# classicvalues/foremast

Measured on AMD Instinct MI355X. Metric: metric windows scored/sec (node) + p50 decision latency, 10k-service canary, higher is better.
Workload: dtype fp32; 1 GPU; global_batch=80000, seq_len=10080, services=10000, metrics=8, current_points_per_window=50, parallelism=dp1, hip_graph=False, tick_mode=front, decision_stream=comm (overlaps next front kernel), front_wgs_per_cu=1:4, comm_overlap=decision + all-gather + host copy of tick k on a comm stream || tick k+1, pipeline_depth=2, publish=graph

## Files before the change

csrc/include/fm_pairwise.h:

```cpp
#pragma once
#include "fm_common.h"

using namespace fm;

namespace {

constexpr float kPad = INFINITY;

template <int K, bool SPLIT = false, bool TAGGED = true, typename T>
__device__ __forceinline__ void bitonic_sort(T (&v)[K], int (&tag)[K]) {
  static_assert(!SPLIT || (K == 2 && TAGGED), "split layout is two tagged 64-lane registers");
  const int lane = lane_id();
#pragma unroll
  for (int size = 2; size <= 64 * K; size <<= 1) {
    const bool tags = TAGGED && (!SPLIT || size > 64);
    if constexpr (SPLIT) {
      if (size == 128) {
#pragma unroll
        for (int k = 0; k < K; ++k) tag[k] = v[k] == kPad ? -1 : k;
      }
    }
#pragma unroll
    for (int stride = size >> 1; stride > 0; stride >>= 1) {
      if (stride >= 64) {
        const int ks = stride / 64;
#pragma unroll
        for (int k = 0; k < K; ++k) {
          const int p = k ^ ks;
          if (p > k) {
// ... 3 lines not shown
            const bool first = (a < b) == asc;
            v[k] = first ? a : b; v[p] = first ? b : a;
            if (tags) {
              const int ta = tag[k], tb = tag[p];
              tag[k] = first ? ta : tb; tag[p] = first ? tb : ta;
            }
          }
        }
      } else {
#pragma unroll
        for (int k = 0; k < K; ++k) {
          const int i = k * 64 + lane;
          const bool asc = (i & size) == 0;
          const bool lower = (lane & stride) == 0;
          const bool keep_min = lower == asc;
          if (tags) cmpx_lane_any(v[k], tag[k], stride, keep_min);
          else cmpx_lane_any(v[k], stride, keep_min);
        }
      }
    }
  }
}

template <int K, bool REDUCE, typename T>
__device__ __forceinline__ int avg_ranks(const T (&v)[K], int n, int (&rank2)[K], bool (&is_end)[K]) {
  const int lane = lane_id();
  bool ne_prev[K];
  unsigned long long tied = 0;
  T last_prev = 0;
#pragma unroll
  for (int k = 0; k < K; ++k) {
    const T prev = lane_prev(v[k], last_prev);
// ... 95 lines not shown
  o[5] = (n1 > 0 && n2 > 0) ? (double)dnum / ((double)n1 * n2) : 0.0;
  o[6] = 0.5 * (double)rps; o[7] = (double)tiew; o[8] = m1; o[9] = m2; o[10] = q1; o[11] = q2;
  o[12] = npos; o[13] = nzero;
}

struct PwNoHook {
  __device__ __forceinline__ void loaded() const {}
  __device__ __forceinline__ void done() const {}
  __device__ __forceinline__ void store(double* __restrict__ o, int n1, int n2, int nw, unsigned r1s, unsigned tie,
                                        int dnum, unsigned rps, unsigned tiew, float m1, float m2, float q1, float q2,
                                        int npos, int nzero) const {
    if (lane_id() == 0) pw_store_suff(o, n1, n2, nw, r1s, tie, dnum, rps, tiew, m1, m2, q1, q2, npos, nzero);
  }
};

template <int K, bool SPLIT = false, class Hook = PwNoHook>
__device__ __forceinline__ void pw_compute(PwIn<K>& in, int n_cur, int n_base, double* __restrict__ o,
                                           Hook hook = Hook()) {
  const int lane = lane_id();
  float (&v)[K] = in.v;
  int tag[K];
  float s1 = 0.f, s2 = 0.f;
  int n1 = 0, n2 = 0;
#pragma unroll
  for (int k = 0; k < K; ++k) {
    const int i = k * 64 + lane;
    int t = SPLIT ? (lane < (k == 0 ? n_cur : n_base) ? k : -1) : (i < n_cur ? 0 : (i < n_cur + n_base ? 1 : -1));
    float x = v[k];
    if (!isfinite(x)) { x = kPad; t = -1; }
    v[k] = x; tag[k] = t;
    if (t == 0) s1 += x;
    if (t == 1) s2 += x;
    n1 += __popcll(__ballot(t == 0));
    n2 += __popcll(__ballot(t == 1));
  }
  const int n = n1 + n2;
  const float m1 = wave_sum_f32_uniform(s1) / (float)(n1 > 0 ? n1 : 1);
  const float m2 = wave_sum_f32_uniform(s2) / (float)(n2 > 0 ? n2 : 1);
  float q1 = 0.f, q2 = 0.f;
#pragma unroll
  for (int k = 0; k < K; ++k) {
    if (tag[k] == 0) { const float d = v[k] - m1; q1 += d * d; }
    if (tag[k] == 1) { const float d = v[k] - m2; q2 += d * d; }
  }
  q1 = wave_sum_f32_uniform(q1); q2 = wave_sum_f32_uniform(q2);

  constexpr int KW = PwIn<K>::KW;
  constexpr unsigned kPadMag = 0x7F800000u;
  unsigned dk[KW];
  const int npair = n_cur < n_base ? n_cur : n_base;
  int nw = 0, npos = 0, nzero = 0;
#pragma unroll
  for (int k = 0; k < KW; ++k) {
    const int j = k * 64 + lane;
    const float xc = in.pc[k], xb = in.pb[k];
    const float dd = xc - xb;
    const bool ok = j < npair && isfinite(xc) && isfinite(xb);
    const bool nz = ok && dd != 0.f, pos = nz && dd > 0.f;
    dk[k] = nz ? ((__float_as_uint(fabsf(dd)) << 1) | (pos ? 1u : 0u)) : (kPadMag << 1);
    nw += __popcll(__ballot(nz));
    npos += __popcll(__ballot(pos));
    nzero += __popcll(__ballot(ok && !nz));
  }

  hook.loaded();
  constexpr long long N = 64LL * K, NW = 64LL * KW;
  constexpr int bTie = pw_bits(N * N * N - N), bR1 = pw_bits(N * (N + 1));
  constexpr int bTiew = pw_bits(NW * NW * NW - NW), bRp = pw_bits(NW * (NW + 1));
  static_assert(bTie <= 32 && bTiew <= 32 && bR1 <= 32 && bRp <= 32, "32-bit sums");
  constexpr bool packA = bTie + bR1 <= 32;
  constexpr bool packB = bTiew + bRp <= 32;
  constexpr bool packC = !packA && !packB && bR1 + bRp <= 32;
  bitonic_sort<K, SPLIT>(v, tag);
  int rk2[K];
  bool en[K];
  const int tie_l = avg_ranks<K, !packA>(v, n, rk2, en);

  unsigned r1x2 = 0;
  int dnum = 0;
  int base12 = 0;
#pragma unroll
  for (int k = 0; k < K; ++k) {
    if (tag[k] == 0) r1x2 += (unsigned)rk2[k];
    const int a12 = wave_incl_sum(tag[k] == 0 ? 1 : (tag[k] == 1 ? (1 << 16) : 0)) + base12;
    base12 = lane_bcast(a12, 63);
    if (en[k] && n1 > 0 && n2 > 0) {
      const int a1 = a12 & 0xFFFF, a2 = a12 >> 16;
      const int dd = abs(__mul24(a1, n2) - __mul24(a2, n1));
// ... 286 lines not shown
```

csrc/kernels/tick_front.hip:

```cpp
#include "fm_pairwise.h"
#include "fm_row_stats.h"

__device__ __attribute__((noinline)) void eval_test_call(int t, const double* __restrict__ o, int min_mw, int min_wil,
                                                         int min_kru, double& pv, double& sv) {
  eval_test(t, o, min_mw, min_wil, min_kru, pv, sv);
}

#ifdef FM_FRONT_TIMING
constexpr int kFtMarks = 4;
__device__ unsigned long long g_front_t[kFtMarks * 8192];
#define FM_FT_MARK(k) \
  do { if (threadIdx.x == 0 && blockIdx.x < 8192) g_front_t[kFtMarks * blockIdx.x + (k)] = __builtin_amdgcn_s_memrealtime(); } while (0)
#define FM_FT_ROWS(n) \
  do { if (threadIdx.x == 0 && blockIdx.x < 8192) g_front_t[kFtMarks * blockIdx.x + 3] = (unsigned long long)(n); } while (0)
#else
#define FM_FT_MARK(k) do {} while (0)
#define FM_FT_ROWS(n) do {} while (0)
#endif

struct FrontArgs {
  int64_t R;
  int nP, scan, T;
  const float* hist;
  int64_t ld_h;
  float* hs;
  const int* rowmap;
  float* cache;
  unsigned* valid;
  unsigned* queue;
  const float* cur;
  int64_t ld_c;
  const float* base;
  int64_t ld_b;
  double* suff;
  int n_cur, n_base;
  float *pvals, *pstats;
  int min_mw, min_wil, min_kru;
};

constexpr int kXcdCtl = 256, kCtlR = 0, kCtlDone = 1, kCtlB = 2, kCtlOn = 31, kCtlT0 = 32, kCtlT1 = 48;
constexpr int64_t kXcdMinRows = 32768;
constexpr int kFracBits = 24;
constexpr double kXcdBand = 1.015, kXcdStep = 3.0;
constexpr int kHistChunk = 1;
__device__ inline int64_t xcd_bound(int64_t R, unsigned f) { return (R * (int64_t)f) >> kFracBits; }

__device__ __attribute__((noinline)) void xcd_rebalance(unsigned* ctl, int xcd, int64_t R) {
  unsigned long long* t0 = reinterpret_cast<unsigned long long*>(ctl + kCtlT0);
  unsigned long long* t1 = reinterpret_cast<unsigned long long*>(ctl + kCtlT1);
  __hip_atomic_store(t1 + xcd, __builtin_amdgcn_s_memrealtime(), __ATOMIC_RELAXED, __HIP_MEMORY_SCOPE_AGENT);
  const unsigned g = __hip_atomic_fetch_add(ctl + kCtlDone, 1u, __ATOMIC_ACQ_REL, __HIP_MEMORY_SCOPE_AGENT);
  if (g != 7u) return;
// ... 70 lines not shown
      uint4* s = reinterpret_cast<uint4*>(raw);
      s[0] = make_uint4((unsigned)n1, (unsigned)n2, (unsigned)nw, r1s);
      s[1] = make_uint4(tie, (unsigned)dnum, rps, tiew);
      s[2] = make_uint4(__float_as_uint(m1), __float_as_uint(m2), __float_as_uint(q1), __float_as_uint(q2));
      *reinterpret_cast<uint2*>(raw + 12) = make_uint2((unsigned)npos, (unsigned)nzero);
    }
  }
};

__device__ __forceinline__ void front_raw_to_suff(const unsigned* __restrict__ raw, double* __restrict__ o) {
  const uint4 a = reinterpret_cast<const uint4*>(raw)[0], b = reinterpret_cast<const uint4*>(raw)[1];
  const uint4 c = reinterpret_cast<const uint4*>(raw)[2];
  const uint2 d = *reinterpret_cast<const uint2*>(raw + 12);
  pw_store_suff(o, (int)a.x, (int)a.y, (int)a.z, a.w, b.x, (int)b.y, b.z, b.w, __uint_as_float(c.x),
                __uint_as_float(c.y), __uint_as_float(c.z), __uint_as_float(c.w), (int)d.x, (int)d.y);
}

template <int K>
__device__ __forceinline__ void pw_row_grab(const float* __restrict__ c, const float* __restrict__ b, int n_cur,
                                            int n_base, unsigned* raw, bool want, unsigned* ctr, unsigned& next) {
  PwIn<K> in;
  if constexpr (K == 2) {
    if (n_cur <= 64 && n_base <= 64) {
      pw_load<K, true>(c, b, n_cur, n_base, in);
      pw_compute<K, true>(in, n_cur, n_base, nullptr, PwGrab{ctr, want, next, raw});
      return;
    }
  }
  pw_load<K>(c, b, n_cur, n_base, in);
  pw_compute<K, false>(in, n_cur, n_base, nullptr, PwGrab{ctr, want, next, raw});
// ... 8 lines not shown
    const int ci = (u >> 1) * 8 + ((u & 1) ? 7 - slot : slot);
    if (ci >= N_TESTS * cpt) break;
    const int tp = ci / cpt;
    const int t = __builtin_amdgcn_readfirstlane((int)((kByCost >> (4 * tp)) & 7u));
    const int j = (ci - tp * cpt) * 64 + lane_id();
    const int64_t row = j < nr ? rowOf(j) : -1;
    if (row >= 0) {
      double pv, sv;
      eval_test_call(t, a.suff + row * kSuff, a.min_mw, a.min_wil, a.min_kru, pv, sv);
      a.pvals[row * N_TESTS + t] = (float)pv;
      a.pstats[row * N_TESTS + t] = (float)sv;
    }
  }
}

template <int K>
__device__ __forceinline__ void front_pairwise_static(const FrontArgs& a, const int pb) {
  const int64_t R = a.R, first = (int64_t)pb * 4, stride = (int64_t)a.nP * 4;
  for (int64_t row = first + wave_id(); row < R; row += stride) {
    pw_row<K>(a.cur + row * a.ld_c, a.base + row * a.ld_b, a.n_cur, a.n_base, a.suff + row * kSuff);
  }
  __syncthreads();
  FM_FT_MARK(2);
  const int64_t span = R > first ? R - first : 0;
  const int nr = (int)(((span + stride - 1) / stride) * 4);
#ifdef FM_FRONT_TIMING
  {
    int64_t took = 0;
    for (int w = 0; w < 4; ++w) took += span > w ? (span - w + stride - 1) / stride : 0;
    FM_FT_ROWS(took);
  }
#endif
  front_pvalues(a, nr, (wave_id() + pb) & 3, [&](int j) {
    const int64_t row = first + (j & 3) + (int64_t)(j >> 2) * stride;
    return row < R ? row : (int64_t)-1;
  });
}

template <int K>
__device__ __forceinline__ void front_pairwise_dyn(const FrontArgs& a, const FrontDyn& dq, const int pb) {
  __shared__ int s_rows[4][kRowCap];
  __shared__ int s_cnt[4];
  __shared__ __attribute__((aligned(16))) unsigned s_raw[4][kRowCap][kRawWords];
  const int w = wave_id(), lane = lane_id();
  const int nP = a.nP, W = nP * 4, Q = dq.q;
  const int x = (pb + pb / Q) % Q;
  const int64_t pool = a.R - dq.pool0;
  const int lo = dq.pool0 + (int)(pool * x / Q), hi = dq.pool0 + (int)(pool * (x + 1) / Q);
  const unsigned nx = (unsigned)(hi - lo);
  unsigned* ctr = dq.pq + x * 32;
  unsigned next = 0;
  bool pending = false;
  if (dq.s == 0 && nx != 0u) {
    unsigned idx = 0;
// ... 7 lines not shown
    int row;
    if (i < dq.s) {
      row = pb * 4 + w + i * W;
    } else {
      if (!pending) break;
      if (next >= nx) break;
      row = lo + (int)next;
    }
    switch ((cls + i) & 3) {
      case 0: __builtin_amdgcn_s_setprio(0); break;
      case 1: __builtin_amdgcn_s_setprio(1); break;
      case 2: __builtin_amdgcn_s_setprio(2); break;
      default: __builtin_amdgcn_s_setprio(3); break;
    }
    const bool want = nx != 0u && i + 1 >= dq.s && i + 1 < kRowCap;
    pw_row_grab<K>(a.cur + (int64_t)row * a.ld_c, a.base + (int64_t)row * a.ld_b, a.n_cur, a.n_base, s_raw[w][i],
                   want, ctr, next);
    pending = want;
    if (lane == 0) s_rows[w][i] = row;
    ++i;
  }
  __builtin_amdgcn_s_setprio(0);
  if (lane == 0) s_cnt[w] = i;
  __syncthreads();
  FM_FT_MARK(2);
  const int c0 = s_cnt[0], c1 = c0 + s_cnt[1], c2 = c1 + s_cnt[2], nr = c2 + s_cnt[3];
  FM_FT_ROWS(nr);
  auto listed = [&](int j, int& ww, int& k) {
    ww = (j >= c0 ? 1 : 0) + (j >= c1 ? 1 : 0) + (j >= c2 ? 1 : 0);
    k = j - (ww == 0 ? 0 : (ww == 1 ? c0 : (ww == 2 ? c1 : c2)));
  };
  if ((int)threadIdx.x < nr) {
// ... 70 lines not shown
    __syncthreads();
    if (threadIdx.x == 0) s_next = nxt;
    __syncthreads();
    r0 = lo + (int64_t)s_next;
  }
  if (threadIdx.x == 0) {
    const unsigned d = atomicAdd(ctr + 1, 1u);
    if (d == (unsigned)nwg - 1) {
      __hip_atomic_store(ctr, 0u, __ATOMIC_RELAXED, __HIP_MEMORY_SCOPE_AGENT);
      __hip_atomic_store(ctr + 1, 0u, __ATOMIC_RELAXED, __HIP_MEMORY_SCOPE_AGENT);
      if (bal) xcd_rebalance(ctl, xcd, R);
    }
  }
}

template <int NV, int K, bool DYN>
__device__ __forceinline__ void tick_front_body(const FrontArgs& a, const FrontDyn& dq) {
  __shared__ double red[4];
  __shared__ int redi[4];
  FM_FT_MARK(0);
  const int nH = (int)gridDim.x - a.nP;
  const int pb = DYN ? (int)blockIdx.x - nH : (int)blockIdx.x;
  const int64_t hb = DYN ? (int64_t)blockIdx.x : (int64_t)blockIdx.x - a.nP;
  if (pb >= 0 && pb < a.nP) {
    if constexpr (DYN) front_pairwise_dyn<K>(a, dq, pb);
    else front_pairwise_static<K>(a, pb);
  } else if (DYN || a.scan) {
    front_hist_scan<NV>(a, hb, nH, red, redi);
  } else if (a.queue == nullptr) {
    front_hist_stride<NV>(a.hist, a.ld_h, a.T, a.R, a.hs, a.rowmap, a.cache, a.valid, hb, nH, red, redi);
  } else {
    front_hist_queue<NV>(a.hist, a.ld_h, a.T, a.R, a.hs, a.rowmap, a.cache, a.valid, a.queue, hb, nH, red, redi);
  }
  FM_FT_MARK(1);
}

template <int NV, int K>
__global__ __launch_bounds__(256) void tick_front_kernel(const FrontArgs a) {
  tick_front_body<NV, K, false>(a, FrontDyn{});
}

template <int NV, int K>
__global__ __launch_bounds__(256) void tick_front_dyn_kernel(const FrontArgs a, const FrontDyn dq) {
  tick_front_body<NV, K, true>(a, dq);
}

struct FrontPlan {
  int nP, s, q;
  int64_t pool0;
};
static FrontPlan front_plan(int64_t R, int nP, int q_ranges, bool scan) {
  static const int share = [] {
    const char* e = getenv("FM_FRONT_DYN_SHARE");
    const int v = e != nullptr ? atoi(e) : -1;
    return v < 0 || v > 100 ? -1 : v;
  }();
  const int64_t pmax = (R + 3) / 4;
  if (nP <= 0 || nP > pmax) nP = (int)pmax;
  const int64_t per0 = R > 0 ? (R + 4 * (int64_t)nP - 1) / (4 * (int64_t)nP) : 0;
// ... 15 lines not shown
FM_API int fm_front_plan(int64_t R, int nP, int q_ranges, int scan, int64_t* out) {
  if (out == nullptr) return (int)hipErrorInvalidValue;
  const FrontPlan p = front_plan(R, nP, q_ranges, scan != 0);
  out[0] = p.s, out[1] = p.pool0, out[2] = p.q, out[3] = p.nP;
  return 0;
}

static unsigned front_lds() {
  static const unsigned b = [] {
    const char* e = getenv("FM_FRONT_LDS");
    return e != nullptr ? (unsigned)atoi(e) : 33u * 1024u;
  }();
  return b;
}

FM_API int fm_tick_front(const float* hist, int64_t ld_h, int T, int64_t R, float* hs, const float* cur, int64_t ld_c,
                         int n_cur, const float* base, int64_t ld_b, int n_base, double* suff, int nP, int nH,
                         int min_mw, int min_wil, int min_kru, float* pvals, float* pstats, unsigned* queue,
                         const int* rowmap, float* cache, unsigned* valid, int expect_miss, unsigned* pqueue,
                         int q_ranges, hipStream_t stream) {
  if (R <= 0) return 0;
  if ((ld_h & 3) != 0 || (((uintptr_t)hist) & 15) != 0) return (int)hipErrorInvalidValue;
  const int n = n_cur + n_base;
  if (base == nullptr || n_base <= 0 || n > 256) return (int)hipErrorInvalidValue;
  if (cache == nullptr || valid == nullptr || T <= 0) cache = nullptr, valid = nullptr;
  const int scan = cache != nullptr && expect_miss == 0 ? 1 : 0;
  const FrontPlan plan = front_plan(R, nP, pqueue != nullptr ? q_ranges : 0, scan != 0);
  if (scan && nH <= 0) nH = (int)((R + 255) / 256);
  if (nH <= 0 || nH > R) nH = (int)R;
  if (!scan && queue != nullptr && nH < 8) nH = 8;
  const int nq = (T + 3) / 4;
  const dim3 grid((unsigned)(plan.nP + nH)), block(256);
  const unsigned lds = scan ? 0u : front_lds();
  const FrontArgs a{R, plan.nP, scan, T, hist, ld_h, hs, rowmap, cache, valid, queue, cur, ld_c, base, ld_b, suff,
                    n_cur, n_base, pvals, pstats, min_mw, min_wil, min_kru};
  const FrontDyn dq{pqueue, plan.q, plan.s, (int)plan.pool0};
  const int rc = row_stats_dispatch_nv(nq, [&](auto nv) {
    auto launch = [&](auto k) {
      constexpr int NV = decltype(nv)::value, K = decltype(k)::value;
      if (plan.q > 0) hipLaunchKernelGGL((tick_front_dyn_kernel<NV, K>), grid, block, lds, stream, a, dq);
      else hipLaunchKernelGGL((tick_front_kernel<NV, K>), grid, block, lds, stream, a);
    };
    if (n <= 64) launch(std::integral_constant<int, 1>{});
    else if (n <= 128) launch(std::integral_constant<int, 2>{});
    else launch(std::integral_constant<int, 4>{});
  });
  if (rc != 0) return rc;
  FM_LAUNCH_CHECK();
  return 0;
}

FM_API int fm_front_timing_read(unsigned long long* host, int n) {
#ifdef FM_FRONT_TIMING
  if (n > kFtMarks * 8192) n = kFtMarks * 8192;
  return (int)hipMemcpyFromSymbol(host, HIP_SYMBOL(g_front_t), (size_t)n * 8, 0, hipMemcpyDeviceToHost);
#else
  (void)host; (void)n;
  return (int)hipErrorNotSupported;
#endif
}
```

foremast_amd/engine/scorer.py:

```python
from __future__ import annotations

import dataclasses
import os
import weakref
from dataclasses import dataclass

import torch

from ..config import BrainConfig
from ..ops import canary as C


@dataclass
class CanaryOutputs:
    pvals: torch.Tensor
    pstats: torch.Tensor
    diff: torch.Tensor
    suff: torch.Tensor
    decide: C.DecideResult
    packed: torch.Tensor
    hs: torch.Tensor | None = None
    effect: torch.Tensor | None = None
    effect_counts: torch.Tensor | None = None
    effect_passed: torch.Tensor | None = None
# ... 12 lines not shown
        self.hist = hist
        self.cache = RowStatsCache(hist.shape[0], hist.device)
        self.version = hist._version

    def expect_miss(self, T: int, rows: int, stream: int | None) -> bool:
        v = self.hist._version
        if v != self.version:
            self.version = v
            if rows == len(self.cache):
                self.cache.dirty = rows
            else:
                self.cache.invalidate(stream)
        return self.cache.expect_miss(T, rows)


class CanaryScorer:

    def __init__(self, aliases: list[str], cfg: BrainConfig | None = None, device="cpu", overlap: bool = True,
                 mode: str | None = None, hist_blocks: int = 0, pw_blocks: int = 0, pw_cap_rows: int = 32,
                 front_wgs: tuple[float, float] | None = None, front_queue: bool = True,
                 xcd_balance: bool | None = None, hist_cache: bool = True,
                 front_hot_wgs: tuple[float, float] | None = None, model: str = "moving_average_all",
                 codes=None, tail_z: float = 2.0):
        self.mode = mode or ("front" if overlap else "serial")
        if self.mode not in MODES:
            raise ValueError(f"mode must be one of {MODES}")
        if model not in MODELS:
            raise ValueError(f"model must be one of {MODELS}")
        self.model = model
        self.robust = model == "robust_moving_average_all"
        self.band = model == "band_mix"
        if (self.robust or self.band) and self.mode == "fused":
            raise ValueError(f"mode='fused' reads mean/std off the row image: not available for model={model!r}")
        if self.band:
            from ..ops import misc as MI
            if codes is None or len(codes) != len(aliases) or any(int(c) not in (0, 1, 2) for c in codes):
                raise ValueError("model='band_mix' takes codes, one of 0, 1, 2 (ops.misc.BAND_CODES) per metric")
            if len(aliases) > MI.BAND_MAX_METRICS:
# ... 21 lines not shown
        if self.mode == "overlap" and self.device.type == "cuda":
            cus = torch.cuda.get_device_properties(self.device).multi_processor_count
            if pw_blocks == 0:
                self.pw_blocks = cus
            if hist_blocks == 0:
                self.hist_blocks = 8 * cus
        self.front_wgs = front_wgs or (1.0, 4.0)
        self._q_ranges = int(os.environ.get("FM_FRONT_DYN_Q", "64")) if self.device.type == "cuda" else 0
        if front_hot_wgs is None:
            front_hot_wgs = tuple(float(x) for x in os.environ.get(
                "FM_FRONT_HOT_WGS", "4:0.25" if self._q_ranges > 0 else "5:0.25").split(":"))
        self.front_hot_wgs = front_hot_wgs
        self.hist_cache = hist_cache and os.environ.get("FM_HIST_CACHE", "1") != "0"
        self._bound: dict[int, _BoundHist] = {}
        self._store_caches = weakref.WeakSet()
        self._queue = (torch.zeros(8 * 32 + 64, dtype=torch.int32, device=self.device)
                       if front_queue and self.device.type == "cuda" else None)
        if xcd_balance is None:
            xcd_balance = os.environ.get("FM_XCD_BALANCE", "1") != "0"
        if self._queue is not None and xcd_balance:
            self._queue[8 * 32 + 31] = 1
        self._pqueue = (torch.zeros(self._q_ranges * 32, dtype=torch.int32, device=self.device)
                        if self._q_ranges > 0 else None)
        self._cus = (torch.cuda.get_device_properties(self.device).multi_processor_count
                     if self.device.type == "cuda" else 0)
        rules = [self.cfg.rule_for(a) for a in aliases]
        self.thr = torch.tensor([r.threshold for r in rules], dtype=torch.float32, device=self.device)
        self.bound = torch.tensor([r.bound for r in rules], dtype=torch.int32, device=self.device)
        self.minlb = torch.tensor([r.min_lower_bound for r in rules], dtype=torch.float32, device=self.device)
        self.pcfg = C.PairwiseConfig(self.cfg.pairwise_algorithm, self.cfg.pairwise_threshold,
# ... 135 lines not shown
        C.check(self.M <= 16, "resident tick supports up to 16 metrics per service")
        o = self._gate_into(cur, None, self._alloc(R, cur.shape[1], slot)) if not has_base \
            else self._alloc(R, cur.shape[1], slot)
        st = stream_of(cur)
        n = cur.shape[1] + (base.shape[1] if has_base else 0)
        if self.robust:
            return self._resident_robust(hview, rowmap, cur, base if has_base else None, o, st)
        if self.band:
            return self._resident_band(hview, rowmap, cur, base if has_base else None, o, st)
        cache = getattr(hview, "cache", None) if self.hist_cache else None
        miss = True
        if cache is not None:
            self._store_caches.add(cache)
            miss = cache.expect_miss(hview.T, R)
        if has_base and n <= 256:
            LIB.call("fm_tick_front",
                     *self._front_args(ptr(hview.hist), hview.ld, hview.T, base, cur, o, rowmap, cache, miss), st)
        else:
            c_stats, c_valid = (ptr(cache.stats), ptr(cache.valid)) if cache is not None else (None, None)
            LIB.call("fm_hist_stats_cached", ptr(hview.hist), hview.ld, hview.T, R, ptr(o.hs), 0, ptr(rowmap),
                     c_stats, c_valid, int(miss), st)
            if has_base and n <= C.PAIRWISE_MAX:
                self._pairwise_into(cur, base, o, combine=False)
            elif has_base:
                p, s_, _ = C.pairwise_tests(cur, base, self.pcfg)
                o.pvals.copy_(p)
                o.pstats.copy_(s_)
        if cache is not None:
            cache.ticked(hview.T)
        if has_base:
            self._gate_into(cur, base, o)
        self._decide_services(cur, o, has_base)
# ... 129 lines not shown
        self._decide_services(cur, o, base is not None)
        if cache is not None:
            cache.ticked(T)
        return o

    def _no_robust(self, what: str) -> None:
        if self.robust or self.band:
            raise ValueError(f"{what} is not available for model={self.model!r}")

    def _front_grid(self, miss: bool) -> tuple[int, int]:
        fp, fh = self.front_wgs if miss else self.front_hot_wgs
        n_p = int(fp * self._cus) if fp > 0 else 0
        n_h = int(fh * self._cus) if fh > 0 else 0
        return n_p, (n_h if miss or fh <= 0 else max(1, n_h))

    def _front_args(self, hist_ptr, ld: int, T: int, base, cur, o: CanaryOutputs, rowmap, cache, miss: bool) -> tuple:
        from ..ops._lib import ptr
        n_p, n_h = self._front_grid(miss)
        c_stats, c_valid = (ptr(cache.stats), ptr(cache.valid)) if cache is not None else (None, None)
        dyn = (ptr(self._pqueue), self._q_ranges) if self._pqueue is not None else (None, 0)
        return (hist_ptr, ld, T, cur.shape[0], ptr(o.hs), ptr(cur), cur.stride(0), cur.shape[1], ptr(base),
                base.stride(0), base.shape[1], ptr(o.suff), n_p, n_h, self.pcfg.min_mann_white, self.pcfg.min_wilcoxon,
                self.pcfg.min_kruskal, ptr(o.pvals), ptr(o.pstats), ptr(self._queue), ptr(rowmap), c_stats, c_valid,
                int(miss), *dyn)

    def _bind(self, hist: torch.Tensor) -> _BoundHist | None:
        if not self.hist_cache:
            return None
        bh = self._bound.get(id(hist))
        if bh is None or bh.hist is not hist:
            bh = self._bound[id(hist)] = _BoundHist(hist)
        return bh

    def invalidate_history(self) -> None:
        for bh in self._bound.values():
            bh.version = -1
        for cache in self._store_caches:
            cache.invalidate()

# ... 23 lines not shown
        T = hist.shape[1] if n_hist is None else int(n_hist)
        R = cur.shape[0]

        def capture(body):
            g = torch.cuda.CUDAGraph()
            s = torch.cuda.Stream(cur.device)
            s.wait_stream(torch.cuda.current_stream(cur.device))
            with torch.cuda.stream(s):
                with torch.cuda.graph(g, stream=s):
                    body()
            torch.cuda.current_stream(cur.device).wait_stream(s)
            return g
        if bh is None:
            return capture(lambda: self.front_only(hist, base, cur, n_hist, packed_out, slot)).replay, o
        from ..ops._lib import LIB, ptr, stream_of
        graphs = {miss: capture(lambda miss=miss: LIB.call(
            "fm_tick_front", *self._front_args(ptr(hist), hist.stride(0), T, base, cur, o, None, bh.cache, miss),
            stream_of(cur))) for miss in (True, False)}

        def replay() -> None:
            graphs[bh.expect_miss(T, R, None)].replay()
            bh.cache.ticked(T)
        return replay, o

    def _decide_services(self, cur, o: CanaryOutputs, has_base: bool) -> None:
        from ..ops._lib import LIB, ptr, stream_of
        C.check(self.M <= 16, "overlap/fused ticks support up to 16 metrics per service (use mode='serial')")
        LIB.call("fm_decide_services_2s" if self.band else "fm_decide_services",
                 *self._decide_call_args(cur, o, has_base), stream_of(cur))

    def _decide_call_args(self, cur, o: CanaryOutputs, has_base: bool) -> tuple:
        from ..ops._lib import ptr
        mask, anyc = self.pcfg.mask_and_combine()
        d = o.decide
        pv = o.pvals if o.pvals_gated is None else o.pvals_gated
        return (ptr(o.bs if self.band else o.hs), ptr(cur), cur.stride(0), cur.shape[1], cur.shape[0] // self.M,
                self.M, ptr(self.thr), ptr(self.bound), ptr(self.minlb), float(self.cfg.pairwise_threshold_factor),
                ptr(pv) if has_base else None, mask, anyc, float(self.pcfg.p_threshold),
                int(self.cfg.min_historical_points), ptr(d.stats), ptr(d.flags), d.flags.shape[1], ptr(d.count),
                ptr(d.score), ptr(d.valid), ptr(o.diff) if has_base else None, ptr(o.packed))

    def _front(self, hist, base, cur, n_hist, o: CanaryOutputs, decide: bool = True) -> None:
        from ..ops._lib import LIB, ptr, stream_of
        T = hist.shape[1] if n_hist is None else int(n_hist)
        C.check(hist.stride(0) % 4 == 0 and hist.data_ptr() % 16 == 0, "history rows must be 16-B aligned")
        LIB.call("fm_tick_front", *self._front_args(ptr(hist), hist.stride(0), T, base, cur, o, None, None, True),
                 stream_of(cur))
        if decide:
            self._gate_into(cur, base, o)
            self._decide_services(cur, o, True)

    def split_launchers(self, hist, base, cur, n_hist=None, packed_out=None, slot: int = 0,
                        front_stream=None, decide_stream=None):
        from ..ops._lib import LIB, ptr
        self._no_robust("split_launchers")
        self._no_gate("split_launchers")
        o = self.front_only(hist, base, cur, n_hist, packed_out, slot)
        torch.cuda.synchronize(cur.device)
        T = hist.shape[1] if n_hist is None else int(n_hist)
        dev = cur.device
        fs = (front_stream or torch.cuda.current_stream(dev)).cuda_stream
        ds = (decide_stream or torch.cuda.current_stream(dev)).cuda_stream
        lib = LIB.load()
        f_fn, d_fn, R = lib.fm_tick_front, lib.fm_decide_services, cur.shape[0]
        d_args = self._decide_call_args(cur, o, True) + (ds,)
        bh = self._bind(hist)
        f_args = {miss: self._front_args(ptr(hist), hist.stride(0), T, base, cur, o, None,
                                         bh.cache if bh is not None else None, miss) + (fs,)
                  for miss in ((True, False) if bh is not None else (True,))}
        expect = bh.expect_miss if bh is not None else (lambda T, R, fs: True)
        ticked = bh.cache.ticked if bh is not None else (lambda T: None)

        def front() -> None:
            rc = f_fn(*f_args[expect(T, R, fs)])
            if rc:
                raise RuntimeError(f"fm_tick_front failed with hipError {rc}")
            ticked(T)

        def decide() -> None:
            rc = d_fn(*d_args)
            if rc:
                raise RuntimeError(f"fm_decide_services failed with hipError {rc}")
        return front, decide, o

    def _fused(self, hist, base, cur, n_hist, o: CanaryOutputs) -> None:
        from ..ops._lib import LIB, ptr, stream_of
        R = cur.shape[0]
        T = hist.shape[1] if n_hist is None else int(n_hist)
        C.check(hist.stride(0) % 4 == 0 and hist.data_ptr() % 16 == 0, "history rows must be 16-B aligned")
        st = stream_of(cur)
        has_base = base is not None
        LIB.call("fm_canary_rows", ptr(hist), hist.stride(0), T, ptr(cur), cur.stride(0), cur.shape[1],
# ... 51 lines not shown
```

foremast_amd/ops/_lib.py:

```python
from __future__ import annotations

import ctypes
import os
from pathlib import Path

import torch

_NATIVE_DIR = Path(__file__).resolve().parent.parent / "_native"
_LIB_PATH = Path(os.environ.get("FOREMAST_HIP_LIB", _NATIVE_DIR / "libforemast_hip.so"))

c_void_p = ctypes.c_void_p
c_int = ctypes.c_int
c_i64 = ctypes.c_int64
c_u32 = ctypes.c_uint32
c_float = ctypes.c_float

_SIGS: dict[str, list] = {
    "fm_pairwise_tests": [c_void_p, c_i64, c_int, c_void_p, c_i64, c_int, c_i64, c_int, c_int, c_float, c_int,
                          c_int, c_int, c_void_p, c_void_p, c_void_p, c_void_p, c_void_p],
    "fm_pairwise_effect": [c_void_p, c_i64, c_int, c_void_p, c_i64, c_int, c_i64, c_float, c_float, c_float, c_int,
                           c_void_p, c_int, c_void_p, c_void_p, c_void_p, c_void_p, c_void_p, c_void_p],
    "fm_stats_decide": [c_void_p, c_i64, c_int, c_void_p, c_i64, c_int, c_i64, c_int, c_void_p, c_void_p, c_void_p,
                        c_float, c_void_p, c_int, c_void_p, c_void_p, c_int, c_void_p, c_void_p, c_void_p, c_void_p],
    "fm_service_reduce": [c_void_p, c_void_p, c_void_p, c_i64, c_int, c_void_p, c_void_p],
# ... 91 lines not shown
    "fm_canary_rows": [c_void_p, c_i64, c_int, c_void_p, c_i64, c_int, c_void_p, c_i64, c_int, c_i64, c_void_p,
                       c_void_p, c_void_p],
    "fm_lsq_project": [c_void_p, c_i64, c_int, c_i64, c_void_p, c_i64, c_void_p, c_void_p, c_void_p, c_void_p,
                       c_void_p],
    "fm_lsq_residual": [c_void_p, c_i64, c_int, c_i64, c_void_p, c_i64, c_void_p, c_void_p, c_void_p, c_void_p],
    "fm_stream_read": [c_void_p, c_i64, c_void_p, c_int, c_void_p],
    "fm_lstm_forward": [c_void_p, c_i64, c_int, c_int, c_void_p, c_void_p, c_void_p, c_void_p, c_void_p, c_void_p,
                        c_void_p],
    "fm_lstm_forward_nct": [c_void_p, c_i64, c_int, c_int, c_void_p, c_void_p, c_void_p, c_void_p, c_void_p,
                            c_void_p, c_int, c_void_p],
    "fm_lstm_forward_v": [c_void_p, c_i64, c_int, c_int, c_void_p, c_void_p, c_void_p, c_void_p, c_void_p,
                          c_void_p, c_int, c_int, c_void_p],
    "fm_tick_front": [c_void_p, c_i64, c_int, c_i64, c_void_p, c_void_p, c_i64, c_int, c_void_p, c_i64, c_int,
                      c_void_p, c_int, c_int, c_int, c_int, c_int, c_void_p, c_void_p, c_void_p, c_void_p,
                      c_void_p, c_void_p, c_int, c_void_p, c_int, c_void_p],
    "fm_front_plan": [c_i64, c_int, c_int, c_int, c_void_p],
    "fm_hist_stats_cached": [c_void_p, c_i64, c_int, c_i64, c_void_p, c_int, c_void_p, c_void_p, c_void_p, c_int,
                             c_void_p],
    "fm_hist_cache_invalidate": [c_void_p, c_i64, c_void_p],
    "fm_copy_d2h_async": [c_void_p, c_void_p, c_i64, c_void_p],
    "fm_memcpy_sync": [c_void_p, c_void_p, c_i64],
    "fm_board_copy": [c_void_p, c_void_p, c_i64],
    "fm_rolling_stats": [c_void_p, c_i64, c_int, c_i64, c_int, c_int, c_void_p, c_void_p, c_i64, c_void_p],
    "fm_pvalues_range": [c_void_p, c_i64, c_int, c_int, c_int, c_int, c_int, c_void_p, c_void_p, c_void_p],
    "fm_lstm_stack": [c_void_p, c_i64, c_int, c_int, c_int, c_void_p, c_void_p, c_void_p, c_void_p, c_int, c_int,
                      c_void_p],
    "fm_lstm_features_mv": [c_void_p, c_i64, c_int, c_i64, c_int, c_int, c_float, c_void_p, c_void_p, c_void_p,
                            c_void_p],
    "fm_lstm_features": [c_void_p, c_i64, c_int, c_i64, c_int, c_float, c_int, c_void_p, c_void_p, c_void_p,
                         c_void_p],
# ... 70 lines not shown
```

Measured before the change: 736.6 million windows/s.

## Cache per-row baseline sort and stats across ticks in split pairwise path

Adds a per-row device cache holding the raw baseline values, the baseline register after its in-register bitonic stages, and the baseline count, mean and variance. Each tick checks the incoming baseline against the cached raw values. On a match it skips the baseline statistics and the intra-register sort stages for that register, and runs only the cross-register merge. This trades extra global loads, a wave-wide compare and cache writes on misses for less sort and reduction work when baselines stay the same between ticks.

After: 809.0 million windows/s, median of 6. 1.1x the previous value.

```diff
diff --git a/csrc/include/fm_pairwise.h b/csrc/include/fm_pairwise.h
--- a/csrc/include/fm_pairwise.h
+++ b/csrc/include/fm_pairwise.h
@@ -7,12 +7,13 @@
 
 constexpr float kPad = INFINITY;
 
-template <int K, bool SPLIT = false, bool TAGGED = true, typename T>
+template <int K, bool SPLIT = false, bool TAGGED = true, int LO = 2, int HI = 64 * K, unsigned REGS = ~0u, typename T>
 __device__ __forceinline__ void bitonic_sort(T (&v)[K], int (&tag)[K]) {
   static_assert(!SPLIT || (K == 2 && TAGGED), "split layout is two tagged 64-lane registers");
+  static_assert(REGS == ~0u || HI <= 64, "a register subset only while no stage crosses registers");
   const int lane = lane_id();
 #pragma unroll
-  for (int size = 2; size <= 64 * K; size <<= 1) {
+  for (int size = LO; size <= HI; size <<= 1) {
     const bool tags = TAGGED && (!SPLIT || size > 64);
     if constexpr (SPLIT) {
       if (size == 128) {
@@ -46,8 +47,12 @@
           const bool asc = (i & size) == 0;
           const bool lower = (lane & stride) == 0;
           const bool keep_min = lower == asc;
-          if (tags) cmpx_lane_any(v[k], tag[k], stride, keep_min);
-          else cmpx_lane_any(v[k], stride, keep_min);
+          if (REGS != ~0u && ((REGS >> k) & 1u) == 0u) {
+          } else if (tags) {
+            cmpx_lane_any(v[k], tag[k], stride, keep_min);
+          } else {
+            cmpx_lane_any(v[k], stride, keep_min);
+          }
         }
       }
     }
@@ -173,36 +178,88 @@
   }
 };
 
-template <int K, bool SPLIT = false, class Hook = PwNoHook>
+struct PwNoBase {
+  static constexpr bool kOn = false;
+};
+struct PwBaseCache {
+  static constexpr bool kOn = true;
+  unsigned* __restrict__ raw;
+  unsigned* __restrict__ sorted;
+  uint4* __restrict__ stats;
+  unsigned row;
+  unsigned r = 0, s = 0;
+  uint4 st = {0u, 0u, 0u, 0u};
+  __device__ __forceinline__ unsigned at() const { return row * 64u + (unsigned)lane_id(); }
+  __device__ __forceinline__ void load(int n_base) {
+    r = lane_id() < n_base ? raw[at()] : 0u;
+    s = sorted[at()];
+    st = stats[row];
+  }
+  __device__ __forceinline__ bool hit(float b, int n_base) const {
+    const bool differs = (lane_id() < n_base && __float_as_uint(b) != r) || st.w != (unsigned)n_base;
+    return __ballot(differs) == 0ull;
+  }
+};
+
+template <int K, bool SPLIT = false, class Hook = PwNoHook, class Base = PwNoBase>
 __device__ __forceinline__ void pw_compute(PwIn<K>& in, int n_cur, int n_base, double* __restrict__ o,
-                                           Hook hook = Hook()) {
+                                           Hook hook = Hook(), Base bc = Base()) {
+  static_assert(!Base::kOn || SPLIT, "the baseline cache belongs to the split layout");
   const int lane = lane_id();
   float (&v)[K] = in.v;
   int tag[K];
   float s1 = 0.f, s2 = 0.f;
-  int n1 = 0, n2 = 0;
-#pragma unroll
-  for (int k = 0; k < K; ++k) {
-    const int i = k * 64 + lane;
-    int t = SPLIT ? (lane < (k == 0 ? n_cur : n_base) ? k : -1) : (i < n_cur ? 0 : (i < n_cur + n_base ? 1 : -1));
-    float x = v[k];
-    if (!isfinite(x)) { x = kPad; t = -1; }
-    v[k] = x; tag[k] = t;
-    if (t == 0) s1 += x;
-    if (t == 1) s2 += x;
-    n1 += __popcll(__ballot(t == 0));
-    n2 += __popcll(__ballot(t == 1));
-  }
-  const int n = n1 + n2;
-  const float m1 = wave_sum_f32_uniform(s1) / (float)(n1 > 0 ? n1 : 1);
-  const float m2 = wave_sum_f32_uniform(s2) / (float)(n2 > 0 ? n2 : 1);
-  float q1 = 0.f, q2 = 0.f;
-#pragma unroll
-  for (int k = 0; k < K; ++k) {
-    if (tag[k] == 0) { const float d = v[k] - m1; q1 += d * d; }
-    if (tag[k] == 1) { const float d = v[k] - m2; q2 += d * d; }
-  }
-  q1 = wave_sum_f32_uniform(q1); q2 = wave_sum_f32_uniform(q2);
+  int n1 = 0, n2 = 0, n;
+  float m1, m2, q1 = 0.f, q2 = 0.f;
+  bool hit = false;
+  if constexpr (Base::kOn) {
+    hit = bc.hit(v[1], n_base);
+    if (!hit && lane < n_base) bc.raw[bc.at()] = __float_as_uint(v[1]);
+  }
+  if (Base::kOn && hit) {
+    if constexpr (Base::kOn) {
+      int t = lane < n_cur ? 0 : -1;
+      float x = v[0];
+      if (!isfinite(x)) { x = kPad; t = -1; }
+      v[0] = x; tag[0] = t; tag[1] = 1;
+      if (t == 0) s1 += x;
+      n1 += __popcll(__ballot(t == 0));
+      m1 = wave_sum_f32_uniform(s1) / (float)(n1 > 0 ? n1 : 1);
+      if (tag[0] == 0) { const float d = v[0] - m1; q1 += d * d; }
+      q1 = wave_sum_f32_uniform(q1);
+      n2 = __builtin_amdgcn_readfirstlane((int)bc.st.x);
+      m2 = __uint_as_float(bc.st.y); q2 = __uint_as_float(bc.st.z);
+      n = n1 + n2;
+      v[1] = __uint_as_float(bc.s);
+      asm volatile("" : "+v"(v[1]));
+    }
+  } else {
+#pragma unroll
+    for (int k = 0; k < K; ++k) {
+      const int i = k * 64 + lane;
+      int t = SPLIT ? (lane < (k == 0 ? n_cur : n_base) ? k : -1) : (i < n_cur ? 0 : (i < n_cur + n_base ? 1 : -1));
+      float x = v[k];
+      if (!isfinite(x)) { x = kPad; t = -1; }
+      v[k] = x; tag[k] = t;
+      if (t == 0) s1 += x;
+      if (t == 1) s2 += x;
+      n1 += __popcll(__ballot(t == 0));
+      n2 += __popcll(__ballot(t == 1));
+    }
+    n = n1 + n2;
+    m1 = wave_sum_f32_uniform(s1) / (float)(n1 > 0 ? n1 : 1);
+    m2 = wave_sum_f32_uniform(s2) / (float)(n2 > 0 ? n2 : 1);
+#pragma unroll
+    for (int k = 0; k < K; ++k) {
+      if (tag[k] == 0) { const float d = v[k] - m1; q1 += d * d; }
+      if (tag[k] == 1) { const float d = v[k] - m2; q2 += d * d; }
+    }
+    q1 = wave_sum_f32_uniform(q1); q2 = wave_sum_f32_uniform(q2);
+    if constexpr (Base::kOn) {
+      if (lane == 0)
+        bc.stats[bc.row] = make_uint4((unsigned)n2, __float_as_uint(m2), __float_as_uint(q2), (unsigned)n_base);
+    }
+  }
 
   constexpr int KW = PwIn<K>::KW;
   constexpr unsigned kPadMag = 0x7F800000u;
@@ -230,7 +287,17 @@
   constexpr bool packA = bTie + bR1 <= 32;
   constexpr bool packB = bTiew + bRp <= 32;
   constexpr bool packC = !packA && !packB && bR1 + bRp <= 32;
-  bitonic_sort<K, SPLIT>(v, tag);
+  if constexpr (Base::kOn) {
+    if (hit) {
+      bitonic_sort<K, SPLIT, true, 2, 64, 1u>(v, tag);
+    } else {
+      bitonic_sort<K, SPLIT, true, 2, 64>(v, tag);
+      bc.sorted[bc.at()] = __float_as_uint(v[1]);
+    }
+    bitonic_sort<K, SPLIT, true, 128, 128>(v, tag);
+  } else {
+    bitonic_sort<K, SPLIT>(v, tag);
+  }
   int rk2[K];
   bool en[K];
   const int tie_l = avg_ranks<K, !packA>(v, n, rk2, en);
diff --git a/csrc/kernels/tick_front.hip b/csrc/kernels/tick_front.hip
--- a/csrc/kernels/tick_front.hip
+++ b/csrc/kernels/tick_front.hip
@@ -36,6 +36,8 @@
   int n_cur, n_base;
   float *pvals, *pstats;
   int min_mw, min_wil, min_kru;
+  unsigned *bc_raw, *bc_sorted;
+  uint4* bc_stats;
 };
 
 constexpr int kXcdCtl = 256, kCtlR = 0, kCtlDone = 1, kCtlB = 2, kCtlOn = 31, kCtlT0 = 32, kCtlT1 = 48;
@@ -136,6 +138,17 @@
   const uint2 d = *reinterpret_cast<const uint2*>(raw + 12);
   pw_store_suff(o, (int)a.x, (int)a.y, (int)a.z, a.w, b.x, (int)b.y, b.z, b.w, __uint_as_float(c.x),
                 __uint_as_float(c.y), __uint_as_float(c.z), __uint_as_float(c.w), (int)d.x, (int)d.y);
+}
+
+template <class Hook>
+__device__ __forceinline__ void pw_row_cached(const FrontArgs& a, int64_t row, double* __restrict__ o, Hook hook) {
+  const float* __restrict__ c = a.cur + row * a.ld_c;
+  const float* __restrict__ b = a.base + row * a.ld_b;
+  PwIn<2> in;
+  pw_load<2, true>(c, b, a.n_cur, a.n_base, in);
+  PwBaseCache bc{a.bc_raw, a.bc_sorted, a.bc_stats, (unsigned)row};
+  bc.load(a.n_base);
+  pw_compute<2, true>(in, a.n_cur, a.n_base, o, hook, bc);
 }
 
 template <int K>
@@ -174,11 +187,12 @@
   }
 }
 
-template <int K>
+template <int K, bool BC>
 __device__ __forceinline__ void front_pairwise_static(const FrontArgs& a, const int pb) {
   const int64_t R = a.R, first = (int64_t)pb * 4, stride = (int64_t)a.nP * 4;
   for (int64_t row = first + wave_id(); row < R; row += stride) {
-    pw_row<K>(a.cur + row * a.ld_c, a.base + row * a.ld_b, a.n_cur, a.n_base, a.suff + row * kSuff);
+    if constexpr (BC) pw_row_cached(a, row, a.suff + row * kSuff, PwNoHook());
+    else pw_row<K>(a.cur + row * a.ld_c, a.base + row * a.ld_b, a.n_cur, a.n_base, a.suff + row * kSuff);
   }
   __syncthreads();
   FM_FT_MARK(2);
@@ -197,7 +211,7 @@
   });
 }
 
-template <int K>
+template <int K, bool BC>
 __device__ __forceinline__ void front_pairwise_dyn(const FrontArgs& a, const FrontDyn& dq, const int pb) {
   __shared__ int s_rows[4][kRowCap];
   __shared__ int s_cnt[4];
@@ -235,8 +249,11 @@
       default: __builtin_amdgcn_s_setprio(3); break;
     }
     const bool want = nx != 0u && i + 1 >= dq.s && i + 1 < kRowCap;
-    pw_row_grab<K>(a.cur + (int64_t)row * a.ld_c, a.base + (int64_t)row * a.ld_b, a.n_cur, a.n_base, s_raw[w][i],
-                   want, ctr, next);
+    if constexpr (BC)
+      pw_row_cached(a, (int64_t)row, nullptr, PwGrab{ctr, want, next, s_raw[w][i]});
+    else
+      pw_row_grab<K>(a.cur + (int64_t)row * a.ld_c, a.base + (int64_t)row * a.ld_b, a.n_cur, a.n_base, s_raw[w][i],
+                     want, ctr, next);
     pending = want;
     if (lane == 0) s_rows[w][i] = row;
     ++i;
@@ -337,7 +354,7 @@
   }
 }
 
-template <int NV, int K, bool DYN>
+template <int NV, int K, bool DYN, bool BC>
 __device__ __forceinline__ void tick_front_body(const FrontArgs& a, const FrontDyn& dq) {
   __shared__ double red[4];
   __shared__ int redi[4];
@@ -346,8 +363,8 @@
   const int pb = DYN ? (int)blockIdx.x - nH : (int)blockIdx.x;
   const int64_t hb = DYN ? (int64_t)blockIdx.x : (int64_t)blockIdx.x - a.nP;
   if (pb >= 0 && pb < a.nP) {
-    if constexpr (DYN) front_pairwise_dyn<K>(a, dq, pb);
-    else front_pairwise_static<K>(a, pb);
+    if constexpr (DYN) front_pairwise_dyn<K, BC>(a, dq, pb);
+    else front_pairwise_static<K, BC>(a, pb);
   } else if (DYN || a.scan) {
     front_hist_scan<NV>(a, hb, nH, red, redi);
   } else if (a.queue == nullptr) {
@@ -358,14 +375,14 @@
   FM_FT_MARK(1);
 }
 
-template <int NV, int K>
+template <int NV, int K, bool BC = false>
 __global__ __launch_bounds__(256) void tick_front_kernel(const FrontArgs a) {
-  tick_front_body<NV, K, false>(a, FrontDyn{});
-}
-
-template <int NV, int K>
+  tick_front_body<NV, K, false, BC>(a, FrontDyn{});
+}
+
+template <int NV, int K, bool BC = false>
 __global__ __launch_bounds__(256) void tick_front_dyn_kernel(const FrontArgs a, const FrontDyn dq) {
-  tick_front_body<NV, K, true>(a, dq);
+  tick_front_body<NV, K, true, BC>(a, dq);
 }
 
 struct FrontPlan {
@@ -411,12 +428,17 @@
   return b;
 }
 
-FM_API int fm_tick_front(const float* hist, int64_t ld_h, int T, int64_t R, float* hs, const float* cur, int64_t ld_c,
-                         int n_cur, const float* base, int64_t ld_b, int n_base, double* suff, int nP, int nH,
-                         int min_mw, int min_wil, int min_kru, float* pvals, float* pstats, unsigned* queue,
-                         const int* rowmap, float* cache, unsigned* valid, int expect_miss, unsigned* pqueue,
-                         int q_ranges, hipStream_t stream) {
+FM_API int fm_tick_front_bc(const float* hist, int64_t ld_h, int T, int64_t R, float* hs, const float* cur,
+                            int64_t ld_c, int n_cur, const float* base, int64_t ld_b, int n_base, double* suff, int nP,
+                            int nH, int min_mw, int min_wil, int min_kru, float* pvals, float* pstats, unsigned* queue,
+                            const int* rowmap, float* cache, unsigned* valid, int expect_miss, unsigned* pqueue,
+                            int q_ranges, unsigned* bc_raw, unsigned* bc_sorted, unsigned* bc_stats,
+                            hipStream_t stream) {
   if (R <= 0) return 0;
+  if ((((uintptr_t)bc_stats) & 15) != 0) return (int)hipErrorInvalidValue;
+  const bool use_bc = bc_raw != nullptr && bc_sorted != nullptr && bc_stats != nullptr && n_cur <= 64 &&
+                      n_base <= 64 && n_cur + n_base > 64 && R <= (int64_t)1 << 25;
+  if (!use_bc) bc_raw = bc_sorted = bc_stats = nullptr;
   if ((ld_h & 3) != 0 || (((uintptr_t)hist) & 15) != 0) return (int)hipErrorInvalidValue;
   const int n = n_cur + n_base;
   if (base == nullptr || n_base <= 0 || n > 256) return (int)hipErrorInvalidValue;
@@ -430,21 +452,34 @@
   const dim3 grid((unsigned)(plan.nP + nH)), block(256);
   const unsigned lds = scan ? 0u : front_lds();
   const FrontArgs a{R, plan.nP, scan, T, hist, ld_h, hs, rowmap, cache, valid, queue, cur, ld_c, base, ld_b, suff,
-                    n_cur, n_base, pvals, pstats, min_mw, min_wil, min_kru};
+                    n_cur, n_base, pvals, pstats, min_mw, min_wil, min_kru, bc_raw, bc_sorted,
+                    reinterpret_cast<uint4*>(bc_stats)};
   const FrontDyn dq{pqueue, plan.q, plan.s, (int)plan.pool0};
   const int rc = row_stats_dispatch_nv(nq, [&](auto nv) {
-    auto launch = [&](auto k) {
+    auto launch = [&](auto k, auto bc) {
       constexpr int NV = decltype(nv)::value, K = decltype(k)::value;
-      if (plan.q > 0) hipLaunchKernelGGL((tick_front_dyn_kernel<NV, K>), grid, block, lds, stream, a, dq);
-      else hipLaunchKernelGGL((tick_front_kernel<NV, K>), grid, block, lds, stream, a);
+      constexpr bool BC = decltype(bc)::value;
+      if (plan.q > 0) hipLaunchKernelGGL((tick_front_dyn_kernel<NV, K, BC>), grid, block, lds, stream, a, dq);
+      else hipLaunchKernelGGL((tick_front_kernel<NV, K, BC>), grid, block, lds, stream, a);
     };
-    if (n <= 64) launch(std::integral_constant<int, 1>{});
-    else if (n <= 128) launch(std::integral_constant<int, 2>{});
-    else launch(std::integral_constant<int, 4>{});
+    if (n <= 64) launch(std::integral_constant<int, 1>{}, std::false_type{});
+    else if (n > 128) launch(std::integral_constant<int, 4>{}, std::false_type{});
+    else if (use_bc) launch(std::integral_constant<int, 2>{}, std::true_type{});
+    else launch(std::integral_constant<int, 2>{}, std::false_type{});
   });
   if (rc != 0) return rc;
   FM_LAUNCH_CHECK();
   return 0;
+}
+
+FM_API int fm_tick_front(const float* hist, int64_t ld_h, int T, int64_t R, float* hs, const float* cur, int64_t ld_c,
+                         int n_cur, const float* base, int64_t ld_b, int n_base, double* suff, int nP, int nH,
+                         int min_mw, int min_wil, int min_kru, float* pvals, float* pstats, unsigned* queue,
+                         const int* rowmap, float* cache, unsigned* valid, int expect_miss, unsigned* pqueue,
+                         int q_ranges, hipStream_t stream) {
+  return fm_tick_front_bc(hist, ld_h, T, R, hs, cur, ld_c, n_cur, base, ld_b, n_base, suff, nP, nH, min_mw, min_wil,
+                          min_kru, pvals, pstats, queue, rowmap, cache, valid, expect_miss, pqueue, q_ranges, nullptr,
+                          nullptr, nullptr, stream);
 }
 
 FM_API int fm_front_timing_read(unsigned long long* host, int n) {
diff --git a/foremast_amd/engine/scorer.py b/foremast_amd/engine/scorer.py
--- a/foremast_amd/engine/scorer.py
+++ b/foremast_amd/engine/scorer.py
@@ -50,6 +50,17 @@
         return self.cache.expect_miss(T, rows)
 
 
+class _BaseCache:
+
+    def __init__(self, rows: int, device):
+        self.raw = torch.zeros((rows, 64), dtype=torch.int32, device=device)
+        self.sorted = torch.zeros((rows, 64), dtype=torch.int32, device=device)
+        self.stats = torch.zeros((rows, 4), dtype=torch.int32, device=device)
+
+    def __len__(self) -> int:
+        return self.raw.shape[0]
+
+
 class CanaryScorer:
 
     def __init__(self, aliases: list[str], cfg: BrainConfig | None = None, device="cpu", overlap: bool = True,
@@ -57,7 +68,7 @@
                  front_wgs: tuple[float, float] | None = None, front_queue: bool = True,
                  xcd_balance: bool | None = None, hist_cache: bool = True,
                  front_hot_wgs: tuple[float, float] | None = None, model: str = "moving_average_all",
-                 codes=None, tail_z: float = 2.0):
+                 codes=None, tail_z: float = 2.0, base_cache: bool = True):
         self.mode = mode or ("front" if overlap else "serial")
         if self.mode not in MODES:
             raise ValueError(f"mode must be one of {MODES}")
@@ -109,6 +120,8 @@
         self.hist_cache = hist_cache and os.environ.get("FM_HIST_CACHE", "1") != "0"
         self._bound: dict[int, _BoundHist] = {}
         self._store_caches = weakref.WeakSet()
+        self.base_cache = base_cache and os.environ.get("FM_BASE_CACHE", "1") != "0"
+        self._base_caches: dict[int, tuple] = {}
         self._queue = (torch.zeros(8 * 32 + 64, dtype=torch.int32, device=self.device)
                        if front_queue and self.device.type == "cuda" else None)
         if xcd_balance is None:
@@ -274,8 +287,9 @@
             self._store_caches.add(cache)
             miss = cache.expect_miss(hview.T, R)
         if has_base and n <= 256:
-            LIB.call("fm_tick_front",
-                     *self._front_args(ptr(hview.hist), hview.ld, hview.T, base, cur, o, rowmap, cache, miss), st)
+            LIB.call("fm_tick_front_bc",
+                     *self._front_args(ptr(hview.hist), hview.ld, hview.T, base, cur, o, rowmap, cache, miss,
+                                       self._base_cache_of(base, cur)), st)
         else:
             c_stats, c_valid = (ptr(cache.stats), ptr(cache.valid)) if cache is not None else (None, None)
             LIB.call("fm_hist_stats_cached", ptr(hview.hist), hview.ld, hview.T, R, ptr(o.hs), 0, ptr(rowmap),
@@ -435,15 +449,35 @@
         n_h = int(fh * self._cus) if fh > 0 else 0
         return n_p, (n_h if miss or fh <= 0 else max(1, n_h))
 
-    def _front_args(self, hist_ptr, ld: int, T: int, base, cur, o: CanaryOutputs, rowmap, cache, miss: bool) -> tuple:
+    def _base_cache_of(self, base: torch.Tensor, cur: torch.Tensor) -> _BaseCache | None:
+        n_cur, n_base = cur.shape[1], base.shape[1]
+        if (not self.base_cache or n_cur > 64 or n_base > 64 or n_cur + n_base <= 64
+                or base.shape[0] < cur.shape[0]):
+            return None
+        key = id(base)
+        ent = self._base_caches.get(key)
+        if ent is not None and ent[0]() is base and len(ent[1]) == base.shape[0]:
+            return ent[1]
+        caches = self._base_caches
+
+        def drop(ref, key=key):
+            if key in caches and caches[key][0] is ref:
+                del caches[key]
+        bc = _BaseCache(base.shape[0], base.device)
+        caches[key] = (weakref.ref(base, drop), bc)
+        return bc
+
+    def _front_args(self, hist_ptr, ld: int, T: int, base, cur, o: CanaryOutputs, rowmap, cache, miss: bool,
+                    bcache: _BaseCache | None = None) -> tuple:
         from ..ops._lib import ptr
         n_p, n_h = self._front_grid(miss)
         c_stats, c_valid = (ptr(cache.stats), ptr(cache.valid)) if cache is not None else (None, None)
         dyn = (ptr(self._pqueue), self._q_ranges) if self._pqueue is not None else (None, 0)
+        bc = (ptr(bcache.raw), ptr(bcache.sorted), ptr(bcache.stats)) if bcache is not None else (None, None, None)
         return (hist_ptr, ld, T, cur.shape[0], ptr(o.hs), ptr(cur), cur.stride(0), cur.shape[1], ptr(base),
                 base.stride(0), base.shape[1], ptr(o.suff), n_p, n_h, self.pcfg.min_mann_white, self.pcfg.min_wilcoxon,
                 self.pcfg.min_kruskal, ptr(o.pvals), ptr(o.pstats), ptr(self._queue), ptr(rowmap), c_stats, c_valid,
-                int(miss), *dyn)
+                int(miss), *dyn, *bc)
 
     def _bind(self, hist: torch.Tensor) -> _BoundHist | None:
         if not self.hist_cache:
@@ -497,13 +531,16 @@
         if bh is None:
             return capture(lambda: self.front_only(hist, base, cur, n_hist, packed_out, slot)).replay, o
         from ..ops._lib import LIB, ptr, stream_of
+        bc = self._base_cache_of(base, cur)
         graphs = {miss: capture(lambda miss=miss: LIB.call(
-            "fm_tick_front", *self._front_args(ptr(hist), hist.stride(0), T, base, cur, o, None, bh.cache, miss),
+            "fm_tick_front_bc", *self._front_args(ptr(hist), hist.stride(0), T, base, cur, o, None, bh.cache, miss, bc),
             stream_of(cur))) for miss in (True, False)}
+        keep = (base, bc)
 
         def replay() -> None:
             graphs[bh.expect_miss(T, R, None)].replay()
             bh.cache.ticked(T)
+        replay.keep = keep
         return replay, o
 
     def _decide_services(self, cur, o: CanaryOutputs, has_base: bool) -> None:
@@ -527,7 +564,7 @@
         from ..ops._lib import LIB, ptr, stream_of
         T = hist.shape[1] if n_hist is None else int(n_hist)
         C.check(hist.stride(0) % 4 == 0 and hist.data_ptr() % 16 == 0, "history rows must be 16-B aligned")
-        LIB.call("fm_tick_front", *self._front_args(ptr(hist), hist.stride(0), T, base, cur, o, None, None, True),
+        LIB.call("fm_tick_front_bc", *self._front_args(ptr(hist), hist.stride(0), T, base, cur, o, None, None, True),
                  stream_of(cur))
         if decide:
             self._gate_into(cur, base, o)
@@ -545,11 +582,13 @@
         fs = (front_stream or torch.cuda.current_stream(dev)).cuda_stream
         ds = (decide_stream or torch.cuda.current_stream(dev)).cuda_stream
         lib = LIB.load()
-        f_fn, d_fn, R = lib.fm_tick_front, lib.fm_decide_services, cur.shape[0]
+        f_fn, d_fn, R = lib.fm_tick_front_bc, lib.fm_decide_services, cur.shape[0]
         d_args = self._decide_call_args(cur, o, True) + (ds,)
         bh = self._bind(hist)
+        bc = self._base_cache_of(base, cur)
+        keep = (base, bc)
         f_args = {miss: self._front_args(ptr(hist), hist.stride(0), T, base, cur, o, None,
-                                         bh.cache if bh is not None else None, miss) + (fs,)
+                                         bh.cache if bh is not None else None, miss, bc) + (fs,)
                   for miss in ((True, False) if bh is not None else (True,))}
         expect = bh.expect_miss if bh is not None else (lambda T, R, fs: True)
         ticked = bh.cache.ticked if bh is not None else (lambda T: None)
@@ -557,8 +596,9 @@
         def front() -> None:
             rc = f_fn(*f_args[expect(T, R, fs)])
             if rc:
-                raise RuntimeError(f"fm_tick_front failed with hipError {rc}")
+                raise RuntimeError(f"fm_tick_front_bc failed with hipError {rc}")
             ticked(T)
+        front.keep = keep
 
         def decide() -> None:
             rc = d_fn(*d_args)
diff --git a/foremast_amd/ops/_lib.py b/foremast_amd/ops/_lib.py
--- a/foremast_amd/ops/_lib.py
+++ b/foremast_amd/ops/_lib.py
@@ -129,6 +129,9 @@
     "fm_tick_front": [c_void_p, c_i64, c_int, c_i64, c_void_p, c_void_p, c_i64, c_int, c_void_p, c_i64, c_int,
                       c_void_p, c_int, c_int, c_int, c_int, c_int, c_void_p, c_void_p, c_void_p, c_void_p,
                       c_void_p, c_void_p, c_int, c_void_p, c_int, c_void_p],
+    "fm_tick_front_bc": [c_void_p, c_i64, c_int, c_i64, c_void_p, c_void_p, c_i64, c_int, c_void_p, c_i64, c_int,
+                         c_void_p, c_int, c_int, c_int, c_int, c_int, c_void_p, c_void_p, c_void_p, c_void_p,
+                         c_void_p, c_void_p, c_int, c_void_p, c_int, c_void_p, c_void_p, c_void_p, c_void_p],
     "fm_front_plan": [c_i64, c_int, c_int, c_int, c_void_p],
     "fm_hist_stats_cached": [c_void_p, c_i64, c_int, c_i64, c_void_p, c_int, c_void_p, c_void_p, c_void_p, c_int,
                              c_void_p],
```
